# dropbox/lepton

Measured on AMD Instinct MI355X. Metric: encode+decode MB/s (JPEG bytes/sec), bit-exact round trip, higher is better.
Workload: dtype int16/u8 (integer coder, no floating point)

## Files before the change

lepton_amd/csrc/lep_dec4.h:

```cpp
#pragma once
#include "lep_v3.h"
#include "lep_enc3.h"

namespace lep4 {
using namespace lep3;

#if LEP_ON_GPU && defined(LEP_MARKS)
#define LEP_MARK(name) __asm__ volatile("; MARK " name)
#elif LEP_ON_GPU && defined(LEP_PROF)
#define LEP_MARK(name) prof_stamp(lep4::prof_slot(name))
#else
#define LEP_MARK(name) ((void)0)
#endif
#if LEP_ON_GPU && (defined(LEP_DEC4_PAD_VALU) || defined(LEP_DEC4_PAD_SALU) || defined(LEP_DEC4_PAD_LDS))
#define LEP_PAD8(x) x x x x x x x x
WDEV void pad_block(uint32_t seed, const void* lds) {
    (void)seed; (void)lds;
#ifdef LEP_DEC4_PAD_VALU
    { uint32_t o; for (int i = 0; i < LEP_DEC4_PAD_VALU / 8; ++i) __asm__ volatile(LEP_PAD8("v_add_u32 %0, %1, %1\n") : "=v"(o) : "v"(seed)); }
#endif
#ifdef LEP_DEC4_PAD_SALU
    { uint32_t o; const uint32_t u = uni(seed); for (int i = 0; i < LEP_DEC4_PAD_SALU / 8; ++i) __asm__ volatile(LEP_PAD8("s_add_u32 %0, %1, %1\n") : "=s"(o) : "s"(u) : "scc"); }
#endif
#ifdef LEP_DEC4_PAD_LDS
// ... 86 lines not shown
        }
        r.mul = q + (rem ? 1u : 0u);
        r.shift = s - 1;
        return r;
    }
};
WDEV uint32_t mulhi_u32(uint32_t a, uint32_t b) {
#if LEP_ON_GPU
    return __umulhi(a, b);
#else
    return (uint32_t)(((uint64_t)a * b) >> 32);
#endif
}
WDEV int32_t div_by(int32_t n, uint32_t mul, uint32_t shift) {
    const int32_t sign = n >> 31;
    const uint32_t u = ((uint32_t)n ^ (uint32_t)sign) - (uint32_t)sign;
    const uint32_t q = mulhi_u32(u, mul) >> shift;
    return (int32_t)((q ^ (uint32_t)sign) - (uint32_t)sign);
}
WDEV uint32_t bupd_t(uint32_t w, uint32_t obs, const uint32_t* inv24) {
    const uint32_t f = (w & 255) + (obs ^ 1), t = ((w >> 8) & 255) + obs;
    uint32_t nw = f | (t << 8) | ((mul24(f << 8, inv24[f + t]) >> 24) << 16);
    if ((f | t) > 255) {
        const uint32_t f0 = w & 255, t0 = (w >> 8) & 255;
        if ((obs ? f0 : t0) == 1) nw = (w & 0xffff) | ((obs ? 0u : 255u) << 16);
        else {
            const uint32_t f2 = obs ? (1 + f0) >> 1 : 129u, t2 = obs ? 129u : (1 + t0) >> 1;
            nw = f2 | (t2 << 8) | ((mul24(f2 << 8, inv24[f2 + t2]) >> 24) << 16);
        }
    }
    return nw;
}
WDEV uint32_t bupd_u(uint32_t w, uint32_t obs, const uint32_t* inv24) {
    const uint32_t w2 = w + 1u + obs * 255u;
    const uint32_t f = w2 & 255u, t = (w2 >> 8) & 255u;
    if (ucond((f < t ? f : t) == 0)) {
        const uint32_t f0 = w & 255, t0 = (w >> 8) & 255;
        if (ucond((obs ? f0 : t0) == 1)) return (w & 0xffff) | ((obs ? 0u : 255u) << 16);
        const uint32_t f2 = obs ? (1 + f0) >> 1 : 129u, t2 = obs ? 129u : (1 + t0) >> 1;
        return f2 | (t2 << 8) | ((mul24(f2 << 8, inv24[f2 + t2]) >> 24) << 16);
    }
    return (w2 & 0xffffu) | (mul24_low(f, inv24[f + t]) & 0xff0000u);
}

WDEV uint64_t pair64(uint32_t hi, uint32_t lo) {
#if LEP_ON_GPU && !defined(LEP_DEC4_PAIR_OR)
    typedef uint32_t u32x2 __attribute__((ext_vector_type(2)));
    const u32x2 p = {lo, hi};
    return __builtin_bit_cast(uint64_t, p);
#else
    return ((uint64_t)hi << 32) | lo;
#endif
}
struct BoolDec4 {
    uint32_t vhi, vlo;
    int count;
    uint32_t range;
    const uint32_t* words;
    uint32_t first, end;
    uint32_t wi;
    uint32_t raw;

    WDEV uint32_t fetch(uint32_t k) const { return k * 4 < end ? words[k] : 0u; }
    WDEV void refill() {
        const uint32_t lo = wi * 4;
        uint32_t w = __builtin_bswap32(raw);
        int nbits = 32;
        if (lo + 4 > end) w = lo < end ? (w & ~(0xffffffffu >> ((end - lo) * 8))) : 0u;
        if (lo < first) { w <<= (first - lo) * 8; nbits -= (int)(first - lo) * 8; }
        const uint64_t add = ((uint64_t)w << 32) >> (count + 8);
        vhi |= (uint32_t)(add >> 32); vlo |= (uint32_t)add;
        count += nbits;
        ++wi;
        raw = fetch(wi);
    }
    WDEV void init_stream(const uint8_t* p, uint32_t n) {
        const uint32_t mis = (uint32_t)((uintptr_t)p & 3);
        words = reinterpret_cast<const uint32_t*>(p - mis);
        first = mis; end = mis + n;
        vhi = vec(0); vlo = vec(0); count = (int)vec((uint32_t)-8); range = vec(255); wi = 0;
        raw = fetch(0);
        refill();
        get(128);
    }
    WDEV uint32_t get(uint32_t prob) {
#if LEP_ON_GPU
        const uint32_t split = 1 + (__umul24(range - 1, prob) >> 8);
#else
        const uint32_t split = 1 + (((range - 1) * prob) >> 8);
#endif
        if (ucond(count < 0)) refill();
        const uint32_t big = split << 24;
        const uint32_t bit = vhi >= big ? 1u : 0u;
        const uint32_t d = vhi - big;
        vhi = d < vhi ? d : vhi;
        range = bit ? range - split : split;
#ifdef LEP_TRACE_GET
        LEP_TRACE_GET(prob, (int)bit);
#endif
        const int shift = __builtin_clz(range) - 24;
        range <<= shift;
        const uint64_t v = pair64(vhi, vlo) << shift;
        vhi = (uint32_t)(v >> 32); vlo = (uint32_t)v;
        count -= shift;
        return bit;
    }
};

struct BoolDec4S {
    uint32_t vhi, vlo;
    int count;
    uint32_t range;
#ifdef LEP_DEC4_RANGE_LOW
    WDEV void load(const BoolDec4& b) { vhi = uni(b.vhi); vlo = uni(b.vlo); count = (int)uni((uint32_t)b.count); range = uni(b.range); }
    WDEV void store(BoolDec4& b) const { b.vhi = vec(vhi); b.vlo = vec(vlo); b.count = (int)vec((uint32_t)count); b.range = vec(range); }
#else
    WDEV void load(const BoolDec4& b) { vhi = uni(b.vhi); vlo = uni(b.vlo); count = (int)uni((uint32_t)b.count); range = uni(b.range) << 24; }
    WDEV void store(BoolDec4& b) const { b.vhi = vec(vhi); b.vlo = vec(vlo); b.count = (int)vec((uint32_t)count); b.range = vec(range >> 24); }
#endif
    WDEV void refill(BoolDec4& b) {
        const uint32_t lo = b.wi * 4;
        uint32_t w = __builtin_bswap32(uni(b.raw));
        int nbits = 32;
        if (lo + 4 > b.end) w = lo < b.end ? (w & ~(0xffffffffu >> ((b.end - lo) * 8))) : 0u;
        if (lo < b.first) { w <<= (b.first - lo) * 8; nbits -= (int)(b.first - lo) * 8; }
        const uint64_t add = ((uint64_t)w << 32) >> (count + 8);
        vhi |= (uint32_t)(add >> 32); vlo |= (uint32_t)add;
        count += nbits;
        ++b.wi;
        b.raw = b.fetch(b.wi);
    }
    WDEV uint32_t get(BoolDec4& b, uint32_t pk) {
        if (count < 0) refill(b);
#ifdef LEP_DEC4_RANGE_LOW
        const uint32_t split = 1 + (((range - 1) * (pk & 255u)) >> 8);
        const uint32_t big = split << 24;
        uint32_t was = vhi;
        const uint32_t bit = was >= big ? 1u : 0u;
        vhi = bit ? was - big : was;
        range = bit ? range - split : split;
        const int shift = __builtin_clz(range) - 24;
#else
        const uint32_t big = ((uint32_t)(((uint64_t)(range - 0x01000000u) * (uint64_t)(pk << 24)) >> 32) & 0xff000000u) + 0x01000000u;
        uint32_t was = vhi;
        const uint32_t bit = was >= big ? 1u : 0u;
        vhi = bit ? was - big : was;
        range = bit ? range - big : big;
        const int shift = __builtin_clz(range);
#endif
#ifdef LEP_TRACE_GET
        LEP_TRACE_GET(pk & 255u, (int)bit);
#endif
        range <<= shift;
        const uint64_t v = pair64(vhi, vlo) << shift;
        vhi = (uint32_t)(v >> 32); vlo = (uint32_t)v;
        count -= shift;
#if LEP_ON_GPU && !defined(LEP_DEC4_PAIR_OR)
        __asm__ volatile("" : "+s"(was));
        return was >= big ? 1u : 0u;
#else
        return bit;
#endif
    }
};

#ifndef LEP_DEC4_PRIO
#define LEP_DEC4_PRIO 1
#endif
#if LEP_ON_GPU && LEP_DEC4_PRIO
#define LEP_PRIO_SERIAL(on_scalar_unit) __builtin_amdgcn_s_setprio((on_scalar_unit) ? 0 : 1)
#define LEP_PRIO_PARALLEL() __builtin_amdgcn_s_setprio(2)
#else
#define LEP_PRIO_SERIAL(on_scalar_unit) ((void)0)
#define LEP_PRIO_PARALLEL() ((void)0)
#endif
#ifndef LEP_DEC4_SCALAR
#define LEP_DEC4_SCALAR 2
#endif

enum : int32_t { kRowsFresh = 0, kRowsRunning = 1, kRowsFinished = 2, kRowsFailed = 3 };
struct Dec4Resume {
    int32_t state, code;
    uint32_t idx, top;
    uint32_t vhi, vlo;
    int32_t count;
    uint32_t range, wi;
    uint32_t nbins;
    int32_t rows_done[3];
    int32_t fail_component, fail_y, fail_x;
};

struct RowsWalk {
    const Dec4Resume* rec; const uint32_t* lds_save;
    bool fresh;
    uint32_t idx, stop, total;
    int band;
    bool top[3];
    int rows_done[3];
    int state, fail_component, fail_y, fail_x;
};

template <int SCMASK>
struct Dec4WaveT {
    const ImageDev* img;
    uint32_t* model;
    Dec4Shared* sh;
    int comp, ci;
    BoolDec4 bc;
    uint32_t nbins;
#if LEP_ON_GPU && !defined(LEP_COUNT_BINS)
#define LEP_BINS(expr) ((void)0)
#else
#define LEP_BINS(expr) (expr)
#endif
#if LEP_ON_GPU && defined(LEP_PROF)
    uint64_t prof_last;
    unsigned long long* prof_out;
    int prof_cur;
    uint32_t prof_acc[20];
    template <int I> __device__ __forceinline__ void prof_add(uint32_t dt) { if (prof_cur == I) prof_acc[I] += dt; }
    __device__ __forceinline__ void prof_stamp(int slot) {
        const uint64_t t = __builtin_readcyclecounter();
        const uint32_t dt = (uint32_t)(t - prof_last);
        prof_last = t;
        prof_add<0>(dt); prof_add<1>(dt); prof_add<2>(dt); prof_add<3>(dt); prof_add<4>(dt); prof_add<5>(dt); prof_add<6>(dt);
        prof_add<7>(dt); prof_add<8>(dt); prof_add<9>(dt); prof_add<10>(dt); prof_add<11>(dt); prof_add<12>(dt); prof_add<13>(dt);
        prof_add<14>(dt); prof_add<15>(dt); prof_add<16>(dt); prof_add<17>(dt); prof_add<18>(dt);
        prof_cur = slot;
    }
    __device__ __forceinline__ void prof_begin(unsigned long long* out) {
        for (int i = 0; i < 20; ++i) prof_acc[i] = 0;
        prof_out = out; prof_cur = 18; prof_last = __builtin_readcyclecounter();
    }
    __device__ __forceinline__ void prof_end() {
        prof_stamp(18);
        if (threadIdx.x == 0) for (int i = 0; i < 19; ++i) prof_out[i] = prof_acc[i];
    }
#endif

    WDEV void init_tables() {
        LANES(l) {
            sh->r2a[l] = kR2A[l]; sh->a2r[l] = kA2R[l]; sh->nzbin[l] = l < 50 ? kNzBin[l] : 9;
            for (int d = l; d < kSignWords; d += 64) sh->sign[d] = kBranchInit;
            for (int d = l; d < kResDcWords; d += 64) sh->resdc[d] = kBranchInit;
            if (l < (int)(sizeof(NSum) / 4)) { ((uint32_t*)&sh->ns_left)[l] = 0; ((uint32_t*)&sh->ns_above)[l] = 0; }
            for (int d = l; d < 512; d += 64) sh->inv24[d] = inv24_of((uint32_t)d);
            if (l < 32) {
                int j = 0, c = l;
                while (j < 6 && c >= 7 - j) { c -= 7 - j; ++j; }
                sh->cj[l] = (uint8_t)(l < 28 ? j : 7); sh->cn[l] = (uint8_t)(l < 28 ? c + 1 : 0);
            }
        }
        LSYNC();
    }
    WDEV void stage_component(int c) {
        comp = c; ci = c ? 1 : 0;
        LANES(l) {
            sh->q[l] = img->q[c][l];
            sh->thr[l] = img->min_thresh[c][l];
            if (l >= 8) { sh->icos_x[l] = img->icos_x[c][l]; sh->icos_y[l] = img->icos_y[c][l]; }
            if (l < 15) {
                const uint32_t d = l < 7 ? (uint32_t)img->icos_x[c][(l + 1) * 8] : (l < 14 ? (uint32_t)img->icos_y[c][(l - 6) * 8] : (uint32_t)img->q[c][0]);
                const DivBy m = DivBy::of(d < 2 || d > 0x7fffffffu ? 2u : d);
                if (l < 7) sh->icos_x[l] = (int32_t)m.mul;
                else if (l < 14) sh->icos_y[l - 7] = (int32_t)m.mul;
                else { sh->icos_x[7] = (int32_t)m.mul; sh->icos_y[7] = d == 1 ? 32 : (int32_t)m.shift; }
            }
        }
        LSYNC();
    }

    template <bool SC>
    struct Serial {
        Dec4WaveT& w;
        BoolDec4S s;
        WDEV explicit Serial(Dec4WaveT& w_) : w(w_) { if (SC) s.load(w.bc); }
        WDEV void done() { if (SC) s.store(w.bc); }
        static WDEV uint32_t U(uint32_t x) { return SC ? uni(x) : vec(x); }
        static WDEV bool is(bool c) { return SC ? c : ucond(c); }
        WDEV uint32_t get(uint32_t prob) { return SC ? s.get(w.bc, prob) : w.bc.get(prob); }
        WDEV uint32_t bupd(uint32_t word, uint32_t obs) {
            if (!SC) return bupd_u(word, obs, w.sh->inv24);
            const uint32_t w2 = word + 1u + obs * 255u;
            const uint32_t f = w2 & 255u, t = (w2 >> 8) & 255u;
            if ((f < t ? f : t) == 0) {
                const uint32_t f0 = word & 255, t0 = (word >> 8) & 255;
                if ((obs ? f0 : t0) == 1) return (word & 0xffff) | ((obs ? 0u : 255u) << 16);
                const uint32_t f2 = obs ? (1 + f0) >> 1 : 129u, t2 = obs ? 129u : (1 + t0) >> 1;
                return f2 | (t2 << 8) | ((((f2 << 8) * uni(w.sh->inv24[f2 + t2])) >> 24) << 16);
            }
            return (w2 & 0xffffu) | ((f * uni(w.sh->inv24[f + t])) & 0xff0000u);
        }
        WDEV uint32_t global_bin(uint32_t idx) {
            const uint32_t word = U(vload(w.model + idx));
            const uint32_t bit = get(word >> 16);
            const uint32_t nw = bupd(word, bit);
#if LEP_ON_GPU
            if (threadIdx.x == 0) w.model[idx] = nw;
#else
            w.model[idx] = nw;
#endif
            return bit;
        }
        template <int K>
        WDEV int unary_from(uint32_t pk) {
            if (K <= 0) { if (!is(get(pk & 255) != 0)) return 0; }
            if (K <= 1) { if (!is(get((pk >> 8) & 255) != 0)) return 1; }
            if (K <= 2) { if (!is(get((pk >> 16) & 255) != 0)) return 2; }
            if (!is(get(pk >> 24) != 0)) return 3;
            return 4;
        }
        WDEV int unary_tail(uint32_t gbase) {
            int i = 8;
#pragma nounroll
            for (; i < 11; ++i) if (!is(global_bin(row_word(gbase, i)) != 0)) break;
            return i;
        }
        WDEV uint32_t residual(uint32_t pk, int b, uint32_t v) {
            if (b >= 3) v |= get(pk >> 24) << 3;
            if (b >= 2) v |= get((pk >> 16) & 255) << 2;
            if (b >= 1) v |= get((pk >> 8) & 255) << 1;
            if (b >= 0) v |= get(pk & 255);
            return v;
        }
        template <int LEVELS>
        WDEV int tree(const uint32_t* PK, int base) {
            uint32_t pk = U(lepwave::wave_read(PK, base));
            uint32_t n = get(pk & 255);
            pk = U(lepwave::wave_read(PK, base + 1));
            n = (n << 1) | get((pk >> (n * 8)) & 255);
            pk = U(lepwave::wave_read(PK, base + 2));
            n = (n << 1) | get((pk >> (n * 8)) & 255);
#pragma unroll
            for (int d = 3; d < LEVELS; ++d) {
                pk = U(lepwave::wave_read(PK, base + (1 << (d - 2)) + 1 + (int)uni(n >> 2)));
                n = (n << 1) | get((pk >> ((n & 3) * 8)) & 255);
            }
            return (int)uni(n);
        }
    };

    static WDEV U4 vload4(const uint32_t* p) {
#if LEP_ON_GPU
        uintptr_t a = (uintptr_t)p;
        __asm__ volatile("" : "+v"(a));
        return ld4(reinterpret_cast<const uint32_t*>(a));
#else
        return ld4(p);
#endif
    }
    static WDEV uint32_t vload(const uint32_t* p) {
#if LEP_ON_GPU
        uintptr_t a = (uintptr_t)p;
        __asm__ volatile("" : "+v"(a));
        return *reinterpret_cast<const uint32_t*>(a);
#else
        return *p;
#endif
    }
    WDEV void idct_rows() { idct_no_dc(sh); }
    static WDEV int half16(int d) { return (int16_t)d / 2; }

    static WDEV void mask_exp(int i0, int len, int& used, int& bits) {
        int n = imin(len, 10) - i0 + 1;
        n = n < 0 ? 0 : (n > 4 ? 4 : n);
        used = (1 << n) - 1;
        const int z = len - i0;
        bits = (z >= 0 && z < 4) ? (used & ~(1 << z)) : used;
    }
    static WDEV void mask_res(int top, int v, int& used, int& bits) {
        top = top > 3 ? 3 : top;
        used = top < 0 ? 0 : (1 << (top + 1)) - 1;
        bits = v & used;
    }
    static WDEV void mask_tree(int i, int k, int value, int& used, int& bits) {
        const int prefix = value >> (i + 1);
        used = (prefix >> 2) == k ? 1 << (prefix & 3) : 0;
        bits = ((value >> i) & 1) ? used : 0;
    }
    template <int ALWAYS>
    WDEV void adapt_group(U4* W, const int* used, const int* bits) {
        const uint32_t* inv = sh->inv24;
#ifdef LEP_DEC4_ADAPT_BRANCHY
        {
            LV(int, any0);
#define LEP_SLOT0(k, fld)                                                                                             \
            LANES(l) L(any0) = (L(used) >> k) & 1;                                                                    \
            if (lepwave::wave_ballot(any0)) {                                                                         \
                LANES(l) if ((L(used) >> k) & 1) L(W).fld = bupd_t(L(W).fld, (uint32_t)(L(bits) >> k) & 1u, inv);    \
            }
            LEP_SLOT0(0, x) LEP_SLOT0(1, y) LEP_SLOT0(2, z) LEP_SLOT0(3, w)
#undef LEP_SLOT0
            return;
        }
#endif
        LV(int, any); LV(uint32_t, oldw); LV(uint32_t, low);
#ifdef LEP_DEC4_ALWAYS_OVERRIDE
        constexpr int kAlways = LEP_DEC4_ALWAYS_OVERRIDE;
#else
        constexpr int kAlways = ALWAYS;
#endif
#define LEP_SLOT(k, fld)                                                                                              \
        if (!((kAlways >> k) & 1)) { LANES(l) L(any) = (L(used) >> k) & 1; }                                           \
        if (((kAlways >> k) & 1) || lepwave::wave_ballot(any)) {                                                       \
            LANES(l) {                                                                                                \
                const uint32_t w = L(W).fld;                                                                          \
                const uint32_t u1 = ((uint32_t)(L(used) & L(bits)) >> k) & 1u, u0 = ((uint32_t)(L(used) & ~L(bits)) >> k) & 1u;   \
                const uint32_t w2 = w + (u0 | (u1 << 8));                                                             \
                const uint32_t f = w2 & 255u, t = (w2 >> 8) & 255u;                                                   \
                const uint32_t p = mul24_low(f, inv[f + t]);    \
                const uint32_t m = mul24(u0 | u1, 0xff0000u);                                                         \
                L(oldw) = w; L(low) = (f < t ? f : t) + ((u0 | u1) ^ 1u);    \
                L(W).fld = (p & m) | (w2 & ~m);                                                                       \
            }                                                                                                         \
            LANES(l) L(any) = L(low) == 0;                                                                            \
            if (lepwave::wave_ballot(any)) {                                                                          \
                LANES(l) if (L(low) == 0) L(W).fld = bupd_t(L(oldw), (uint32_t)(L(bits) >> k) & 1u, inv);             \
            }                                                                                                         \
        }
        LEP_SLOT(0, x) LEP_SLOT(1, y) LEP_SLOT(2, z) LEP_SLOT(3, w)
#undef LEP_SLOT
    }

    WDEV int round_nz(int nzbin_ctx) {
        LEP_MARK("nz_prefetch");
        LV(U4, W0); LV(uint32_t, a0); LV(uint32_t, PK0);
        LANES(l) {
            uint32_t adr = 0, pk = 0;
            if (l < 17) {
                int i, k;
                if (l < 3) { i = 5 - l; k = 0; } else if (l < 5) { i = 2; k = l - 3; } else if (l < 9) { i = 1; k = l - 5; } else { i = 0; k = l - 9; }
                adr = ctx_nz7(ci, nzbin_ctx) + (uint32_t)i * 32 + (uint32_t)k * 4;
                L(W0) = ld4(model + adr); pk = pack_probs(L(W0));
            }
            L(a0) = adr; L(PK0) = pk;
        }
        LEP_MARK("nz_serial"); LEP_PRIO_SERIAL((SCMASK & 1) != 0);
        int nz;
        {
            Serial<(SCMASK & 1) != 0> sr(*this);
            nz = sr.template tree<6>(PK0, 0);
            sr.done();
            LEP_BINS(nbins += 6);
        }
        LEP_MARK("nz_update"); LEP_PRIO_PARALLEL();
        LV(int, u0); LV(int, b0);
        LANES(l) {
            int u = 0, b = 0;
            if (l < 17) {
                int i, k;
                if (l < 3) { i = 5 - l; k = 0; } else if (l < 5) { i = 2; k = l - 3; } else if (l < 9) { i = 1; k = l - 5; } else { i = 0; k = l - 9; }
                mask_tree(i, k, nz, u, b);
            }
            L(u0) = u; L(b0) = b;
        }
        adapt_group<3>(W0, u0, b0);
        LANES(l) if (L(u0)) st4(model + L(a0), L(W0));
        return nz;
    }

    WDEV void round_77(int& zz_io, int& left_io) {
        Dec4Shared& S = *sh;
        LEP_MARK("77_prefetch");
        const int zz0 = zz_io, left0 = left_io, nb0 = nzbin_of(left0);
        LV(U4, W0); LV(U4, W1); LV(uint32_t, a0); LV(uint32_t, a1); LV(uint32_t, PK0); LV(uint32_t, PK1); LV(int, ok);
        LANES(l) {
            const int pi = l & 15, cand = l >> 4, p = zz0 + pi, nb = nb0 - cand;
            uint32_t adr0 = 0, adr1 = 0, pk0 = 0, pk1 = 0;
            const int valid = p < 49 && nb >= 1 && cand < LEP_DEC4_CANDS && pi >= left0 - nzhi_of(nb < 0 ? 0 : nb);
            if (valid) {
                adr0 = ctx4_exp7(ci, nb, p, S.bsr[p]);
                adr1 = ctx4_res(ci, S.a2r[p], nb);
                L(W0) = ld4(model + adr0);
                pk0 = pack_probs(L(W0));
                L(W1) = ld4(model + adr1); pk1 = pack_probs(L(W1));

            }
            L(a0) = adr0; L(a1) = adr1; L(PK0) = pk0; L(PK1) = pk1; L(ok) = valid;
        }
        LSYNC();
        LEP_MARK("77_serial"); LEP_PRIO_SERIAL((SCMASK & 2) != 0);
        int zz, left = left0, cand = 0;
        const int pi_end = zz0 + 16 < 49 ? 16 : 49 - zz0;
        {
            typedef Serial<(SCMASK & 2) != 0> SR;
            SR sr(*this);
            uint32_t sgw = SR::U(S.sign[ci * 48]);
            int pi = 0;
#pragma nounroll
            for (;;) {
                int lane = pi + 16 * cand;
                const int lane_end = pi_end + 16 * cand;
                uint32_t pkv;
                bool found = false;
#pragma nounroll
                for (;;) {
                    pkv = SR::U(lepwave::wave_read(PK0, lane));
                    LEP_BINS(++nbins);
                    if (SR::is(sr.get(pkv & 255) != 0)) { found = true; break; }
                    if (++lane >= lane_end) break;
                }
                pi = lane - 16 * cand;
                if (!found) break;
                zz = zz0 + pi;
                int len = sr.template unary_from<1>(pkv);
                if (len == 4) {
                    len = 4 + sr.template unary_from<0>(SR::U(pack_probs(vload4(model + ctx4_exp7(ci, nb0 - cand, zz, (int)uni(S.bsr[zz])) + kGS))));
                    if (len == 8) len = sr.unary_tail(ctx4_exp7(ci, nb0 - cand, zz, (int)uni(S.bsr[zz])));
                }
                LEP_BINS(nbins += (uint32_t)(2 * len - (len == 11)));
                const uint32_t pos = sr.get(sgw >> 16);
                sgw = sr.bupd(sgw, pos);
                --left;
                uint32_t v = 1u << (len - 1);
                if (len > 1) {
                    int b = len - 2;
                    if (b >= 4) {
                        const uint32_t rbase = ctx4_res(ci, (int)uni(S.a2r[zz]), nb0 - cand);
#pragma nounroll
                        for (; b >= 4; --b) v |= sr.global_bin(row_word(rbase, b)) << b;
                    }
                    v = sr.residual(SR::U(lepwave::wave_read(PK1, lane)), b, v);
                }
                S.here[zz] = (int16_t)(pos ? (int)v : -(int)v);
                ++pi;
                if (left == 0) break;
                cand = nb0 - nzbin_of(left);
                if (cand >= LEP_DEC4_CANDS || pi >= pi_end) break;
            }
            zz = zz0 + pi;
            sr.done();
            S.sign[ci * 48] = sgw;
        }
        LSYNC();
        LEP_MARK("77_update"); LEP_PRIO_PARALLEL();
        LV(int, nzw);
        LANES(l) L(nzw) = l < 16 && zz0 + l < zz && S.here[zz0 + l] != 0;
        const uint32_t nzmask = (uint32_t)lepwave::wave_ballot(nzw);
        LV(int, u0); LV(int, b0); LV(int, u1); LV(int, b1); LV(int, u2); LV(int, b2);
        LANES(l) {
            int ua = 0, ba = 0, ub = 0, bb = 0, uc = 0, bcc = 0;
            const int pi = l & 15, cand_l = l >> 4, p = zz0 + pi;
            if (L(ok) && p < zz) {
                const int left_at = left0 - __builtin_popcount(nzmask & ((1u << pi) - 1));
                if (left_at > 0 && nb0 - (int)S.nzbin[left_at] == cand_l) {
                    const int cf = S.here[p];
                    const int v = cf < 0 ? -cf : cf, len = bitlen((uint32_t)v);
                    mask_exp(0, len, ua, ba);
                    mask_res(len - 2, v, ub, bb);
                    mask_exp(4, len, uc, bcc);
                }
            }
            L(u0) = ua; L(b0) = ba; L(u1) = ub; L(b1) = bb; L(u2) = uc; L(b2) = bcc;
        }
        adapt_group<3>(W0, u0, b0);
        adapt_group<0>(W1, u1, b1);
        LANES(l) {
            if (L(u0)) st4(model + L(a0), L(W0));
            if (L(u1)) st4(model + L(a1), L(W1));
        }
        if (lepwave::wave_ballot(u2)) {
            LV(U4, W2);
            LANES(l) if (L(u2)) L(W2) = ld4(model + L(a0) + kGS);
            adapt_group<0>(W2, u2, b2);
            LANES(l) if (L(u2)) st4(model + L(a0) + kGS, L(W2));
        }
        LSYNC();
        zz_io = zz; left_io = left;
    }

    WDEV int round_edges(int nz, int eob_x, int eob_y, bool has_left, bool has_above) {
        Dec4Shared& S = *sh;
        LEP_MARK("edge_prefetch");
        LV(U4, W0); LV(U4, W1); LV(U4, W2); LV(uint32_t, a0); LV(uint32_t, a2); LV(uint32_t, PK0); LV(uint32_t, PK1); LV(uint32_t, PK2);
        LV(uint32_t, INFO);
        LANES(l) {
            uint32_t adr0 = 0, adr2 = 0, pk0 = 0, pk1 = 0, pk2 = 0, info = 0;
            if (l < 56) {
                const int e = l >= 28 ? 1 : 0, c = l - e * 28, j = S.cj[c], n = S.cn[c];
                const bool horizontal = e == 0;
                const int coord = horizontal ? j + 1 : (j + 1) * 8;
                const int32_t prior = S.eprior[e * 7 + j];
                const uint32_t ap = prior < 0 ? 0u - (uint32_t)prior : (uint32_t)prior;
                const int bsr = bitlen(ap > 1023 ? 1023 : ap);
                adr0 = ctx4_expx(ci, n, horizontal ? j : j + 7, bsr);
                adr2 = ctx4_res(ci, coord, n);
                L(W0) = ld4(model + adr0); L(W2) = ld4(model + adr2);
                pk0 = pack_probs(L(W0)); pk2 = pack_probs(L(W2));
                L(W1) = U4{0, 0, 0, 0};
                const int16_t p16 = (int16_t)prior;
                const int thr = S.thr[coord];
                const uint32_t tctx = (uint32_t)imin((int)((ap & 0xffff) >> thr), 255);
                info = (uint32_t)((ci * 4 + (p16 == 0 ? 0 : (p16 > 0 ? 1 : 2))) * 12 + bsr) | ((uint32_t)thr << 8) | (tctx << 16) |
                       ((uint32_t)bsr << 24) | ((S.eprior[14] >> (e * 7 + j)) & 1 ? 0x80000000u : 0u);
            } else if (l < 62) {
                const int e = l >= 59 ? 1 : 0, lv = l - 56 - 3 * e;
                adr0 = ctx_nzedge(e == 0, ci, e == 0 ? eob_x : eob_y, (nz + 3) / 7) + (uint32_t)(2 - lv) * 4;
                L(W0) = ld4(model + adr0); pk0 = pack_probs(L(W0));
            }
            L(a0) = adr0; L(a2) = adr2; L(PK0) = pk0; L(PK1) = pk1; L(PK2) = pk2; L(INFO) = info;
        }
        LSYNC();
        LEP_MARK("edge_serial"); LEP_PRIO_SERIAL((SCMASK & 4) != 0);
        int ne[2] = {0, 0}, rc = 0;
        typedef Serial<(SCMASK & 4) != 0> SR;
        SR sr(*this);
#pragma nounroll
        for (int e = 0; e < 2 && !rc; ++e) {
            const bool horizontal = e == 0;
            ne[e] = sr.template tree<3>(PK0, 56 + 3 * e);
            LEP_BINS(nbins += 3);
            int left = ne[e];
            if (!left) continue;
            const int a_off = horizontal ? 50 : 57;
            int lane = e * 28 + left - 1, step = 7;
#pragma nounroll
            for (;;) {
                if (SR::is(left > step)) {
#pragma nounroll
                    for (int j = 7 - step; j < 7 && left; ++j) {
                        const uint32_t info = lepwave::wave_read(INFO, e * 28 + combo_base(j));
                        if (info >> 31) { rc = 43; break; }
                        const int coord = horizontal ? j + 1 : (j + 1) * 8;
                        const uint32_t gb = ctx4_expx(ci, left, horizontal ? j : j + 7, (int)((info >> 24) & 15));
                        int len = 0;
#pragma nounroll
                        for (; len < 11; ++len) if (!SR::is(sr.global_bin(row_word(gb, len)) != 0)) break;
                        LEP_BINS(nbins += (uint32_t)(len ? 2 * len + 1 - (len == 11) : 1));
                        if (!len) continue;
                        const int sslot = (int)(info & 255);
                        const uint32_t sgw = SR::U(S.sign[sslot]);
                        const uint32_t pos = sr.get(sgw >> 16);
                        S.sign[sslot] = sr.bupd(sgw, pos);
                        uint32_t v = 1u << (len - 1);
                        int b = len - 2;
                        const int thr = (int)((info >> 8) & 15);
                        if (b >= thr) {
                            const uint32_t Tt = ctx_thresh(ci, (int)((info >> 16) & 255), imin(len - thr, 7));
                            int sx = 1;
#pragma nounroll
                            for (; b >= thr; --b) {
                                const uint32_t bit = sr.global_bin(Tt + (uint32_t)sx);
                                v |= bit << b;
                                sx = imin((sx << 1) | (int)uni(bit), 127);
                            }
                        }
                        const uint32_t rbase = ctx4_res(ci, coord, left);
#pragma nounroll
                        for (; b >= 0; --b) v |= sr.global_bin(row_word(rbase, b)) << b;
                        S.here[a_off + j] = (int16_t)(pos ? (int)v : -(int)v);
                        --left;
                    }
                    break;
                }
                const uint32_t info = lepwave::wave_read(INFO, lane);
                if (info >> 31) { rc = 43; break; }
                const uint32_t pkv = SR::U(lepwave::wave_read(PK0, lane));
                LEP_BINS(++nbins);
                if (SR::is(sr.get(pkv & 255) != 0)) {
                    const int j = 7 - step;
                    const int coord = horizontal ? j + 1 : (j + 1) * 8;
                    int len = sr.template unary_from<1>(pkv);
                    if (len == 4) {
                        len = 4 + sr.template unary_from<0>(SR::U(pack_probs(vload4(model + ctx4_expx(ci, left, horizontal ? j : j + 7, (int)((info >> 24) & 15)) + kGS))));
                        if (len == 8) len = sr.unary_tail(ctx4_expx(ci, left, horizontal ? j : j + 7, (int)((info >> 24) & 15)));
                    }
                    LEP_BINS(nbins += (uint32_t)(2 * len - (len == 11)));
                    const int sslot = (int)(info & 255);
                    const uint32_t sgw = SR::U(S.sign[sslot]);
                    const uint32_t pos = sr.get(sgw >> 16);
                    S.sign[sslot] = sr.bupd(sgw, pos);
                    uint32_t v = 1u << (len - 1);
                    if (len > 1) {
                        int b = len - 2;
                        const int thr = (int)((info >> 8) & 15);
                        if (b >= thr) {
                            const uint32_t Tt = ctx_thresh(ci, (int)((info >> 16) & 255), imin(len - thr, 7));
                            int sx = 1;
#pragma nounroll
                            for (; b >= thr; --b) {
                                const uint32_t bit = sr.global_bin(Tt + (uint32_t)sx);
                                v |= bit << b;
                                sx = imin((sx << 1) | (int)uni(bit), 127);
                            }
                        }
                        if (b >= 4) {
                            const uint32_t rbase = ctx4_res(ci, coord, left);
#pragma nounroll
                            for (; b >= 4; --b) v |= sr.global_bin(row_word(rbase, b)) << b;
                        }
                        v = sr.residual(SR::U(lepwave::wave_read(PK2, lane)), b, v);
                    }
                    S.here[a_off + j] = (int16_t)(pos ? (int)v : -(int)v);
                    --lane;
                    if (--left == 0) break;
                }
                lane += step;
                if (--step == 0) break;
            }
        }
        sr.done();
        LSYNC();
        if (rc) return rc;
        LEP_MARK("edge_update"); LEP_PRIO_PARALLEL();
        LV(int, enz);
        LANES(l) L(enz) = l >= 50 && S.here[l] != 0;
        const uint64_t em = lepwave::wave_ballot(enz);
        const uint32_t mh = (uint32_t)(em >> 50) & 0x7f, mv = (uint32_t)(em >> 57) & 0x7f;
        const int neh = ne[0], nev = ne[1];
        LV(int, u0); LV(int, b0); LV(int, u1); LV(int, b1); LV(int, u2); LV(int, b2);
        LANES(l) {
            int ua = 0, ba = 0, ub = 0, bb = 0, uc = 0, bcc = 0;
            if (l < 56) {
                const int e = l >= 28 ? 1 : 0, c = l - e * 28, j = S.cj[c], n = S.cn[c];
                const uint32_t mk = e ? mv : mh;
                const int left_at = (e ? nev : neh) - __builtin_popcount(mk & ((1u << j) - 1));
                if (left_at == n) {
                    const int cf = S.here[(e ? 57 : 50) + j];
                    const int v = cf < 0 ? -cf : cf, len = bitlen((uint32_t)v);
                    mask_exp(0, len, ua, ba);
                    mask_exp(4, len, ub, bb);
                    mask_res(imin(len - 2, (int)S.thr[e ? (j + 1) * 8 : j + 1] - 1), v, uc, bcc);
                }
            } else if (l < 62) {
                const int e = l >= 59 ? 1 : 0, lv = l - 56 - 3 * e;
                mask_tree(2 - lv, 0, e ? nev : neh, ua, ba);
            }
            L(u0) = ua; L(b0) = ba; L(u1) = ub; L(b1) = bb; L(u2) = uc; L(b2) = bcc;
        }
        adapt_group<3>(W0, u0, b0);
        LANES(l) if (L(u0)) st4(model + L(a0), L(W0));
        if (lepwave::wave_ballot(u1)) {
            LANES(l) if (L(u1)) L(W1) = ld4(model + L(a0) + kGS);
            adapt_group<0>(W1, u1, b1);
            LANES(l) if (L(u1)) st4(model + L(a0) + kGS, L(W1));
        }
        if (lepwave::wave_ballot(u2)) {
            adapt_group<0>(W2, u2, b2);
            LANES(l) if (L(u2)) st4(model + L(a2), L(W2));
        }
        LSYNC();
        return 0;
    }

    WDEV void round_dc(int pred, int a, int b17, int sctx) {
        Dec4Shared& S = *sh;
        LEP_MARK("dc_prefetch");
        LV(U4, W0); LV(uint32_t, a0); LV(uint32_t, PK0); LV(uint32_t, RW);
        LANES(l) {
            uint32_t adr = 0, pk = 0, rw = 0;
            if (l < 3) { adr = ctx_expdc(a, b17) + (uint32_t)l * 4; L(W0) = ld4(model + adr); pk = pack_probs(L(W0)); }
            else if (l < 13) rw = S.resdc[a * 12 + (l - 3)];
            L(a0) = adr; L(PK0) = pk; L(RW) = rw;
        }
        LEP_MARK("dc_serial"); LEP_PRIO_SERIAL((SCMASK & 8) != 0);
        const int sslot = ci * 48 + sctx;
        typedef Serial<(SCMASK & 8) != 0> SR;
        SR sr(*this);
        int len = sr.template unary_from<0>(SR::U(lepwave::wave_read(PK0, 0)));
        if (len == 4) {
            len += sr.template unary_from<0>(SR::U(lepwave::wave_read(PK0, 1)));
            if (len == 8) {
                uint32_t pk = SR::U(lepwave::wave_read(PK0, 2));
#pragma nounroll
                for (; len < 11; ++len) { if (!SR::is(sr.get(pk & 255) != 0)) break; pk >>= 8; }
            }
        }
        LEP_BINS(nbins += (uint32_t)(len ? 2 * len + 1 - (len == 11) : 1));
        uint32_t v = 0, pos = 1;
        if (len) {
            const uint32_t sgw = SR::U(S.sign[sslot]);
            pos = sr.get(sgw >> 16);
            S.sign[sslot] = sr.bupd(sgw, pos);
            v = 1u << (len - 1);
#pragma nounroll
            for (int i = len - 2; i >= 0; --i) v |= sr.get(SR::U(lepwave::wave_read(RW, 3 + i)) >> 16) << i;
        }
        sr.done();
        v = vec(v);
        int d = (int16_t)(pos ? (int)v : -(int)v);
        int dc = d + pred;
        dc = dc < -1024 ? dc + 2049 : dc;
        dc = dc > 1024 ? dc - 2049 : dc;
        S.here[49] = (int16_t)dc;
        LSYNC();
        LEP_MARK("dc_update"); LEP_PRIO_PARALLEL();
        LV(uint32_t, VV); LV(int, u0); LV(int, b0);
        LANES(l) L(VV) = v;
        LANES(l) {
            int u = 0, b = 0;
            if (l < 3) mask_exp(l * 4, len, u, b);
            L(u0) = u; L(b0) = b;
        }
        adapt_group<7>(W0, u0, b0);
        LANES(l) {
            if (L(u0)) st4(model + L(a0), L(W0));
            if (l >= 3 && l < 13 && l - 3 <= len - 2) S.resdc[a * 12 + (l - 3)] = bupd_t(L(RW), (L(VV) >> (l - 3)) & 1u, S.inv24);
        }
        LSYNC();
    }

    WDEV int decode_block(bool has_left, bool has_above) {
        Dec4Shared& S = *sh;
        LEP_MARK("prologue");
        LANES(l) {
            S.here[l] = 0;
            if (l < 49) {
                int prior;
                if (has_left && has_above) prior = (uint16_t)((iabs(S.left[l]) + iabs(S.above[l])) * 13 + 6 * iabs(S.aleft[l])) >> 5;
                else if (has_left) prior = (int16_t)iabs(S.left[l]);
                else if (has_above) prior = (int16_t)iabs(S.above[l]);
                else prior = 0;
                S.bsr[l] = (uint8_t)bitlen((uint32_t)imin(iabs(prior), 1023));
            }
        }
        int nzctx = 0;
        if (has_left && has_above) nzctx = (S.ns_above.nz + S.ns_left.nz + 2) / 4;
        else if (has_above) nzctx = (S.ns_above.nz + 1) / 2;
        else if (has_left) nzctx = (S.ns_left.nz + 1) / 2;
        const int nzbin_ctx = (int)uni((uint32_t)nzbin_of(nzctx));
        LSYNC();

        const int nz = round_nz(nzbin_ctx);
        if (nz > 49) return 7;
        {
            int zz = 0, left = nz;
#pragma nounroll
            while (zz < 49 && left > 0) round_77(zz, left);
        }
        LEP_MARK("lakhani");
        int eob_x, eob_y;
        {
            LV(int, tx); LV(int, ty); LV(int, badf);
            LANES(l) {
                int ex = 0, ey = 0, bad = 0;
                if (l < 49 && S.here[l] != 0) { const int coord = S.a2r[l]; ex = coord & 7; ey = coord >> 3; }
                if (l < 14) {
                    const bool hz = l < 7;
                    const int j = hz ? l : l - 7;
                    const int coord = hz ? j + 1 : (j + 1) * 8;
                    int32_t prior = 0;
                    if (hz ? has_above : has_left) {
                        const int16_t* nbr = hz ? S.above : S.left;
                        const int32_t* icos = hz ? S.icos_x + coord * 8 : S.icos_y + coord;
                        const int step = hz ? 8 : 1;
                        if (icos[0] != 0) {
                            uint32_t acc = (uint32_t)(int32_t)nbr[S.r2a[coord]] * (uint32_t)icos[0];
                            for (int i = 1; i < 8; ++i) {
                                int32_t xi = S.here[S.r2a[coord + i * step]], ai = nbr[S.r2a[coord + i * step]];
                                int32_t term = (i & 1) ? xi + ai : xi - ai;
                                acc -= (uint32_t)icos[i] * (uint32_t)term;
// ... 180 lines not shown
```

lepton_amd/csrc/lep_wave.h:

```cpp
#pragma once
#include <stdint.h>

#if defined(__HIPCC__)
#define LEP_ON_GPU 1
#define LEP_NL 1
#define LEP_LI(l) 0
static __device__ __forceinline__ int lep_lane_now() { int v = (int)(threadIdx.x & 63); __asm__ volatile("" : "+v"(v)); return v; }
#define LANES(l) for (int l = lep_lane_now(), lep_once_ = 1; lep_once_; lep_once_ = 0)
#define WSYNC() __syncthreads()
#define LSYNC() do { __builtin_amdgcn_fence(__ATOMIC_SEQ_CST, "wavefront"); __builtin_amdgcn_wave_barrier(); } while (0)
#define WDEV __device__ __forceinline__
#else
#define LEP_ON_GPU 0
#define LEP_NL 64
#define LEP_LI(l) (l)
static inline int lep_lane_id(int i) { __asm__ volatile("" : "+r"(i)); return i; }
#define LANES(l) for (int lep_i_ = 0; lep_i_ < 64; ++lep_i_) for (int l = lep_lane_id(lep_i_), lep_once_ = 1; lep_once_; lep_once_ = 0)
#define WSYNC() ((void)0)
#define LSYNC() ((void)0)
#define WDEV inline
#endif

#define LV(T, name) T name[LEP_NL]
#define L(name) name[LEP_LI(l)]
// ... 43 lines not shown
#else
    int s = 0;
    for (int i = 0; i < 64; ++i) { int v = in[i]; out[i] = s; s += v; }
    return s;
#endif
}
WDEV int wave_sum(const int* in) {
#if LEP_ON_GPU
    return __builtin_amdgcn_readlane(wave_incl_sum(in[0]), 63);
#else
    int s = 0;
    for (int i = 0; i < 64; ++i) s += in[i];
    return s;
#endif
}

WDEV int wave_max(const int* in) {
#if LEP_ON_GPU
    return __builtin_amdgcn_readlane(wave_incl_max(in[0]), 63);
#else
    int m = in[0];
    for (int i = 1; i < 64; ++i) m = in[i] > m ? in[i] : m;
    return m;
#endif
}

WDEV void wave_prefix_max(const int* in, int* out) {
#if LEP_ON_GPU
    out[0] = wave_incl_max(in[0]);
#else
    int m = in[0];
    for (int i = 0; i < 64; ++i) { m = in[i] > m ? in[i] : m; out[i] = m; }
#endif
}
WDEV void wave_suffix_min(const int* in, int* out) {
#if LEP_ON_GPU
    const int rev = (63 - (int)(threadIdx.x & 63)) * 4;
    const int r = __builtin_amdgcn_ds_bpermute(rev, -in[0]);
    out[0] = -__builtin_amdgcn_ds_bpermute(rev, wave_incl_max(r));
#else
    int m = in[63];
    for (int i = 63; i >= 0; --i) { m = in[i] < m ? in[i] : m; out[i] = m; }
#endif
}

WDEV uint32_t wave_read(const uint32_t* v, int src) {
#if LEP_ON_GPU
    return (uint32_t)__builtin_amdgcn_readlane((int)v[0], src);
#else
    return v[src];
#endif
}

WDEV void wave_write(uint32_t* v, int dst, uint32_t value) {
#if LEP_ON_GPU
    v[0] = (int)(threadIdx.x & 63) == dst ? value : v[0];
#else
    v[dst] = value;
#endif
}

WDEV void wave_select(uint32_t* v, uint64_t m, uint32_t value) {
#if LEP_ON_GPU
    __asm__("v_cndmask_b32_e64 %0, %0, %1, %2" : "+v"(v[0]) : "v"(value), "s"(m));
#else
    for (int i = 0; i < 64; ++i) if ((m >> i) & 1ull) v[i] = value;
#endif
}
WDEV int popc64(uint64_t m) { return __builtin_popcountll(m); }

#if LEP_ON_GPU
template <class T> WDEV T gld(const T* p) { return *(const __attribute__((address_space(1))) T*)(uintptr_t)p; }
template <class T> WDEV void gst(T* p, const T& v) { *(__attribute__((address_space(1))) T*)(uintptr_t)p = v; }
#else
template <class T> WDEV T gld(const T* p) { return *p; }
template <class T> WDEV void gst(T* p, const T& v) { *p = v; }
#endif

WDEV int mbcnt(uint64_t m, int l) {
#if LEP_ON_GPU
    (void)l;
    return (int)__builtin_amdgcn_mbcnt_hi((uint32_t)(m >> 32), __builtin_amdgcn_mbcnt_lo((uint32_t)m, 0u));
#else
    return __builtin_popcountll(m & ((1ull << l) - 1));
#endif
}

}
```

Before: 1578.

## Batch bool-decoder refills per bin group and adapt model words one per lane

The arithmetic decoder now refills whenever fewer than 24 bits remain, with one check before each group of up to three or four bins (unary runs, residuals, tree levels), instead of testing for refill before every bin. Separately, model adaptation after the nz, 7x7, edge and DC rounds no longer updates whole 4-word groups per lane. Each lane instead gathers its single word via ds_bpermute, adapts it, and stores it with a scalar store. Both aim to shorten the serial decode critical path and the vector update work. The cost is extra cross-lane permutes and more complex lane-mapping logic, which must remain bit-exact.

```diff
diff --git a/lepton_amd/csrc/lep_dec4.h b/lepton_amd/csrc/lep_dec4.h
--- a/lepton_amd/csrc/lep_dec4.h
+++ b/lepton_amd/csrc/lep_dec4.h
@@ -162,6 +162,9 @@
     return ((uint64_t)hi << 32) | lo;
 #endif
 }
+#ifndef LEP_DEC4_REFILL_GROUPS
+#define LEP_DEC4_REFILL_GROUPS 1
+#endif
 struct BoolDec4 {
     uint32_t vhi, vlo;
     int count;
@@ -191,15 +194,24 @@
         vhi = vec(0); vlo = vec(0); count = (int)vec((uint32_t)-8); range = vec(255); wi = 0;
         raw = fetch(0);
         refill();
-        get(128);
-    }
-    WDEV uint32_t get(uint32_t prob) {
+        ensure();
+        get_raw(128);
+    }
+    WDEV void ensure() {
+#if LEP_DEC4_REFILL_GROUPS
+        if (ucond(count < 24)) refill();
+#endif
+    }
+    WDEV uint32_t get(uint32_t prob) { ensure(); return get_raw(prob); }
+    WDEV uint32_t get_raw(uint32_t prob) {
 #if LEP_ON_GPU
         const uint32_t split = 1 + (__umul24(range - 1, prob) >> 8);
 #else
         const uint32_t split = 1 + (((range - 1) * prob) >> 8);
 #endif
+#if !LEP_DEC4_REFILL_GROUPS
         if (ucond(count < 0)) refill();
+#endif
         const uint32_t big = split << 24;
         const uint32_t bit = vhi >= big ? 1u : 0u;
         const uint32_t d = vhi - big;
@@ -240,8 +252,20 @@
         ++b.wi;
         b.raw = b.fetch(b.wi);
     }
-    WDEV uint32_t get(BoolDec4& b, uint32_t pk) {
+    WDEV void ensure(BoolDec4& b) {
+#if LEP_DEC4_REFILL_GROUPS
+        if (count < 24) refill(b);
+#else
+        (void)b;
+#endif
+    }
+    WDEV uint32_t get(BoolDec4& b, uint32_t pk) { ensure(b); return get_raw(b, pk); }
+    WDEV uint32_t get_raw(BoolDec4& b, uint32_t pk) {
+#if !LEP_DEC4_REFILL_GROUPS
         if (count < 0) refill(b);
+#else
+        (void)b;
+#endif
 #ifdef LEP_DEC4_RANGE_LOW
         const uint32_t split = 1 + (((range - 1) * (pk & 255u)) >> 8);
         const uint32_t big = split << 24;
@@ -286,6 +310,10 @@
 #endif
 #ifndef LEP_DEC4_SCALAR
 #define LEP_DEC4_SCALAR 2
+#endif
+
+#ifndef LEP_DEC4_WORD_PER_LANE
+#define LEP_DEC4_WORD_PER_LANE 1
 #endif
 
 enum : int32_t { kRowsFresh = 0, kRowsRunning = 1, kRowsFinished = 2, kRowsFailed = 3 };
@@ -389,6 +417,8 @@
         static WDEV uint32_t U(uint32_t x) { return SC ? uni(x) : vec(x); }
         static WDEV bool is(bool c) { return SC ? c : ucond(c); }
         WDEV uint32_t get(uint32_t prob) { return SC ? s.get(w.bc, prob) : w.bc.get(prob); }
+        WDEV void ensure() { if (SC) s.ensure(w.bc); else w.bc.ensure(); }
+        WDEV uint32_t get_raw(uint32_t prob) { return SC ? s.get_raw(w.bc, prob) : w.bc.get_raw(prob); }
         WDEV uint32_t bupd(uint32_t word, uint32_t obs) {
             if (!SC) return bupd_u(word, obs, w.sh->inv24);
             const uint32_t w2 = word + 1u + obs * 255u;
@@ -412,12 +442,14 @@
 #endif
             return bit;
         }
-        template <int K>
+        template <int K, bool ENSURE = true>
         WDEV int unary_from(uint32_t pk) {
-            if (K <= 0) { if (!is(get(pk & 255) != 0)) return 0; }
-            if (K <= 1) { if (!is(get((pk >> 8) & 255) != 0)) return 1; }
-            if (K <= 2) { if (!is(get((pk >> 16) & 255) != 0)) return 2; }
-            if (!is(get(pk >> 24) != 0)) return 3;
+            static_assert(ENSURE || K >= 1, "four bins need a refill test of their own");
+            if (ENSURE) ensure();
+            if (K <= 0) { if (!is(get_raw(pk & 255) != 0)) return 0; }
+            if (K <= 1) { if (!is(get_raw((pk >> 8) & 255) != 0)) return 1; }
+            if (K <= 2) { if (!is(get_raw((pk >> 16) & 255) != 0)) return 2; }
+            if (!is(get_raw(pk >> 24) != 0)) return 3;
             return 4;
         }
         WDEV int unary_tail(uint32_t gbase) {
@@ -427,24 +459,27 @@
             return i;
         }
         WDEV uint32_t residual(uint32_t pk, int b, uint32_t v) {
-            if (b >= 3) v |= get(pk >> 24) << 3;
-            if (b >= 2) v |= get((pk >> 16) & 255) << 2;
-            if (b >= 1) v |= get((pk >> 8) & 255) << 1;
-            if (b >= 0) v |= get(pk & 255);
+            if (b >= 3) { ensure(); v |= get_raw(pk >> 24) << 3; }
+            if (b >= 2) v |= get_raw((pk >> 16) & 255) << 2;
+            if (b >= 1) v |= get_raw((pk >> 8) & 255) << 1;
+            if (b >= 0) v |= get_raw(pk & 255);
             return v;
         }
         template <int LEVELS>
         WDEV int tree(const uint32_t* PK, int base) {
+            static_assert(LEVELS <= 6, "one refill test per three levels");
             uint32_t pk = U(lepwave::wave_read(PK, base));
-            uint32_t n = get(pk & 255);
+            ensure();
+            uint32_t n = get_raw(pk & 255);
             pk = U(lepwave::wave_read(PK, base + 1));
-            n = (n << 1) | get((pk >> (n * 8)) & 255);
+            n = (n << 1) | get_raw((pk >> (n * 8)) & 255);
             pk = U(lepwave::wave_read(PK, base + 2));
-            n = (n << 1) | get((pk >> (n * 8)) & 255);
+            n = (n << 1) | get_raw((pk >> (n * 8)) & 255);
+            if (LEVELS > 3) ensure();
 #pragma unroll
             for (int d = 3; d < LEVELS; ++d) {
                 pk = U(lepwave::wave_read(PK, base + (1 << (d - 2)) + 1 + (int)uni(n >> 2)));
-                n = (n << 1) | get((pk >> ((n & 3) * 8)) & 255);
+                n = (n << 1) | get_raw((pk >> ((n & 3) * 8)) & 255);
             }
             return (int)uni(n);
         }
@@ -532,6 +567,39 @@
 #undef LEP_SLOT
     }
 
+    WDEV void adapt_words(uint32_t* W, const int* use, const int* obs) {
+        const uint32_t* inv = sh->inv24;
+        LV(int, wrapped); LV(uint32_t, oldw);
+        LANES(l) {
+            const uint32_t w = L(W);
+            const uint32_t u = (uint32_t)L(use), u1 = u & (uint32_t)L(obs), u0 = u & ~(uint32_t)L(obs);
+            const uint32_t w2 = w + (u0 | (u1 << 8));
+            const uint32_t f = w2 & 255u, t = (w2 >> 8) & 255u;
+            const uint32_t p = mul24_low(f, inv[f + t]);
+            const uint32_t m = mul24(u, 0xff0000u);
+            L(oldw) = w; L(wrapped) = (f < t ? f : t) + (u ^ 1u) == 0;
+            L(W) = (p & m) | (w2 & ~m);
+        }
+        if (lepwave::wave_ballot(wrapped)) {
+            LANES(l) if (L(wrapped)) L(W) = bupd_t(L(oldw), (uint32_t)L(obs), inv);
+        }
+    }
+    static WDEV void regroup(const U4* G, const int* src, const int* slot, uint32_t* out) {
+        LV(uint32_t, c0); LV(uint32_t, c1); LV(uint32_t, c2); LV(uint32_t, c3);
+        LV(uint32_t, g0); LV(uint32_t, g1); LV(uint32_t, g2); LV(uint32_t, g3);
+        LANES(l) { L(c0) = L(G).x; L(c1) = L(G).y; L(c2) = L(G).z; L(c3) = L(G).w; }
+        lepwave::wave_gather(c0, src, g0); lepwave::wave_gather(c1, src, g1);
+        lepwave::wave_gather(c2, src, g2); lepwave::wave_gather(c3, src, g3);
+        LANES(l) { const int k = L(slot); L(out) = k == 0 ? L(g0) : (k == 1 ? L(g1) : (k == 2 ? L(g2) : L(g3))); }
+    }
+    WDEV void adapt_regrouped(const U4* G, const uint32_t* adr, const int* src, const int* slot, const int* use, const int* obs) {
+        LV(uint32_t, Wd); LV(uint32_t, ad);
+        regroup(G, src, slot, Wd);
+        lepwave::wave_gather(adr, src, ad);
+        adapt_words(Wd, use, obs);
+        LANES(l) if (L(use)) model[L(ad) + (uint32_t)L(slot)] = L(Wd);
+    }
+
     WDEV int round_nz(int nzbin_ctx) {
         LEP_MARK("nz_prefetch");
         LV(U4, W0); LV(uint32_t, a0); LV(uint32_t, PK0);
@@ -554,6 +622,16 @@
             LEP_BINS(nbins += 6);
         }
         LEP_MARK("nz_update"); LEP_PRIO_PARALLEL();
+#if LEP_DEC4_WORD_PER_LANE
+        {
+            LV(int, src); LV(int, slot); LV(int, use); LV(int, ob);
+            LANES(l) {
+                const int t = l < 6 ? l : 0, i = 5 - t, prefix = nz >> (i + 1);
+                L(src) = ((0x953210 >> (4 * t)) & 15) + (prefix >> 2); L(slot) = prefix & 3; L(use) = l < 6; L(ob) = (nz >> i) & 1;
+            }
+            adapt_regrouped(W0, a0, src, slot, use, ob);
+        }
+#else
         LV(int, u0); LV(int, b0);
         LANES(l) {
             int u = 0, b = 0;
@@ -566,6 +644,7 @@
         }
         adapt_group<3>(W0, u0, b0);
         LANES(l) if (L(u0)) st4(model + L(a0), L(W0));
+#endif
         return nz;
     }
 
@@ -573,7 +652,10 @@
         Dec4Shared& S = *sh;
         LEP_MARK("77_prefetch");
         const int zz0 = zz_io, left0 = left_io, nb0 = nzbin_of(left0);
-        LV(U4, W0); LV(U4, W1); LV(uint32_t, a0); LV(uint32_t, a1); LV(uint32_t, PK0); LV(uint32_t, PK1); LV(int, ok);
+        LV(U4, W0); LV(U4, W1); LV(uint32_t, a0); LV(uint32_t, a1); LV(uint32_t, PK0); LV(uint32_t, PK1);
+#if !LEP_DEC4_WORD_PER_LANE
+        LV(int, ok);
+#endif
         LANES(l) {
             const int pi = l & 15, cand = l >> 4, p = zz0 + pi, nb = nb0 - cand;
             uint32_t adr0 = 0, adr1 = 0, pk0 = 0, pk1 = 0;
@@ -586,7 +668,10 @@
                 L(W1) = ld4(model + adr1); pk1 = pack_probs(L(W1));
 
             }
-            L(a0) = adr0; L(a1) = adr1; L(PK0) = pk0; L(PK1) = pk1; L(ok) = valid;
+            L(a0) = adr0; L(a1) = adr1; L(PK0) = pk0; L(PK1) = pk1;
+#if !LEP_DEC4_WORD_PER_LANE
+            L(ok) = valid;
+#endif
         }
         LSYNC();
         LEP_MARK("77_serial"); LEP_PRIO_SERIAL((SCMASK & 2) != 0);
@@ -613,7 +698,7 @@
                 pi = lane - 16 * cand;
                 if (!found) break;
                 zz = zz0 + pi;
-                int len = sr.template unary_from<1>(pkv);
+                int len = sr.template unary_from<1, false>(pkv);
                 if (len == 4) {
                     len = 4 + sr.template unary_from<0>(SR::U(pack_probs(vload4(model + ctx4_exp7(ci, nb0 - cand, zz, (int)uni(S.bsr[zz])) + kGS))));
                     if (len == 8) len = sr.unary_tail(ctx4_exp7(ci, nb0 - cand, zz, (int)uni(S.bsr[zz])));
@@ -648,6 +733,28 @@
         LANES(l) L(nzw) = l < 16 && zz0 + l < zz && S.here[zz0 + l] != 0;
         const uint32_t nzmask = (uint32_t)lepwave::wave_ballot(nzw);
         LV(int, u0); LV(int, b0); LV(int, u1); LV(int, b1); LV(int, u2); LV(int, b2);
+#if LEP_DEC4_WORD_PER_LANE
+        LV(int, src); LV(int, slot);
+        LANES(l) {
+            int s = l, ua = 0, oa = 0, ub = 0, ob = 0, uc = 0, bcc = 0;
+            const int pi = l & 15, k = l >> 4, p = zz0 + pi;
+            if (p < zz) {
+                const int left_at = left0 - __builtin_popcount(nzmask & ((1u << pi) - 1));
+                const int c = left_at > 0 ? nb0 - (int)S.nzbin[left_at] : LEP_DEC4_CANDS;
+                if (c < LEP_DEC4_CANDS) {
+                    const int cf = S.here[p];
+                    const int v = cf < 0 ? -cf : cf, len = bitlen((uint32_t)v);
+                    s = pi + 16 * c;
+                    ua = k <= len; oa = len != k;
+                    ub = k <= len - 2; ob = (v >> k) & 1;
+                    if (c == k) mask_exp(4, len, uc, bcc);
+                }
+            }
+            L(src) = s; L(slot) = k; L(u0) = ua; L(b0) = oa; L(u1) = ub; L(b1) = ob; L(u2) = uc; L(b2) = bcc;
+        }
+        adapt_regrouped(W0, a0, src, slot, u0, b0);
+        if (lepwave::wave_ballot(u1)) adapt_regrouped(W1, a1, src, slot, u1, b1);
+#else
         LANES(l) {
             int ua = 0, ba = 0, ub = 0, bb = 0, uc = 0, bcc = 0;
             const int pi = l & 15, cand_l = l >> 4, p = zz0 + pi;
@@ -669,6 +776,7 @@
             if (L(u0)) st4(model + L(a0), L(W0));
             if (L(u1)) st4(model + L(a1), L(W1));
         }
+#endif
         if (lepwave::wave_ballot(u2)) {
             LV(U4, W2);
             LANES(l) if (L(u2)) L(W2) = ld4(model + L(a0) + kGS);
@@ -770,7 +878,7 @@
                 if (SR::is(sr.get(pkv & 255) != 0)) {
                     const int j = 7 - step;
                     const int coord = horizontal ? j + 1 : (j + 1) * 8;
-                    int len = sr.template unary_from<1>(pkv);
+                    int len = sr.template unary_from<1, false>(pkv);
                     if (len == 4) {
                         len = 4 + sr.template unary_from<0>(SR::U(pack_probs(vload4(model + ctx4_expx(ci, left, horizontal ? j : j + 7, (int)((info >> 24) & 15)) + kGS))));
                         if (len == 8) len = sr.unary_tail(ctx4_expx(ci, left, horizontal ? j : j + 7, (int)((info >> 24) & 15)));
@@ -818,7 +926,10 @@
         const uint64_t em = lepwave::wave_ballot(enz);
         const uint32_t mh = (uint32_t)(em >> 50) & 0x7f, mv = (uint32_t)(em >> 57) & 0x7f;
         const int neh = ne[0], nev = ne[1];
-        LV(int, u0); LV(int, b0); LV(int, u1); LV(int, b1); LV(int, u2); LV(int, b2);
+        LV(int, u1); LV(int, b1); LV(int, u2); LV(int, b2);
+#if !LEP_DEC4_WORD_PER_LANE
+        LV(int, u0); LV(int, b0);
+#endif
         LANES(l) {
             int ua = 0, ba = 0, ub = 0, bb = 0, uc = 0, bcc = 0;
             if (l < 56) {
@@ -828,18 +939,50 @@
                 if (left_at == n) {
                     const int cf = S.here[(e ? 57 : 50) + j];
                     const int v = cf < 0 ? -cf : cf, len = bitlen((uint32_t)v);
+#if !LEP_DEC4_WORD_PER_LANE
                     mask_exp(0, len, ua, ba);
+#endif
                     mask_exp(4, len, ub, bb);
                     mask_res(imin(len - 2, (int)S.thr[e ? (j + 1) * 8 : j + 1] - 1), v, uc, bcc);
                 }
-            } else if (l < 62) {
+            }
+#if !LEP_DEC4_WORD_PER_LANE
+            else if (l < 62) {
                 const int e = l >= 59 ? 1 : 0, lv = l - 56 - 3 * e;
                 mask_tree(2 - lv, 0, e ? nev : neh, ua, ba);
             }
-            L(u0) = ua; L(b0) = ba; L(u1) = ub; L(b1) = bb; L(u2) = uc; L(b2) = bcc;
-        }
+            L(u0) = ua; L(b0) = ba;
+#else
+            (void)ua; (void)ba;
+#endif
+            L(u1) = ub; L(b1) = bb; L(u2) = uc; L(b2) = bcc;
+        }
+#if LEP_DEC4_WORD_PER_LANE
+        {
+            LV(int, src); LV(int, slot); LV(int, use); LV(int, ob);
+            LANES(l) {
+                int s = l, k = l & 3, u = 0, o = 0;
+                if (l < 56) {
+                    const int q = l >> 2, e = q >= 7 ? 1 : 0, j = q - 7 * e;
+                    const int left_at = (e ? nev : neh) - __builtin_popcount((e ? mv : mh) & ((1u << j) - 1));
+                    if (left_at >= 1 && left_at <= 7 - j) {
+                        const int cf = S.here[(e ? 57 : 50) + j];
+                        const int v = cf < 0 ? -cf : cf, len = bitlen((uint32_t)v);
+                        s = e * 28 + ((j * (15 - j)) >> 1) + left_at - 1;
+                        u = k <= len; o = len != k;
+                    }
+                } else if (l < 62) {
+                    const int e = l >= 59 ? 1 : 0, i = 2 - (l - 56 - 3 * e), value = e ? nev : neh;
+                    k = (value >> (i + 1)) & 3; u = 1; o = (value >> i) & 1;
+                }
+                L(src) = s; L(slot) = k; L(use) = u; L(ob) = o;
+            }
+            adapt_regrouped(W0, a0, src, slot, use, ob);
+        }
+#else
         adapt_group<3>(W0, u0, b0);
         LANES(l) if (L(u0)) st4(model + L(a0), L(W0));
+#endif
         if (lepwave::wave_ballot(u1)) {
             LANES(l) if (L(u1)) L(W1) = ld4(model + L(a0) + kGS);
             adapt_group<0>(W1, u1, b1);
@@ -872,8 +1015,9 @@
             len += sr.template unary_from<0>(SR::U(lepwave::wave_read(PK0, 1)));
             if (len == 8) {
                 uint32_t pk = SR::U(lepwave::wave_read(PK0, 2));
-#pragma nounroll
-                for (; len < 11; ++len) { if (!SR::is(sr.get(pk & 255) != 0)) break; pk >>= 8; }
+                sr.ensure();
+#pragma nounroll
+                for (; len < 11; ++len) { if (!SR::is(sr.get_raw(pk & 255) != 0)) break; pk >>= 8; }
             }
         }
         LEP_BINS(nbins += (uint32_t)(len ? 2 * len + 1 - (len == 11) : 1));
@@ -895,8 +1039,29 @@
         S.here[49] = (int16_t)dc;
         LSYNC();
         LEP_MARK("dc_update"); LEP_PRIO_PARALLEL();
-        LV(uint32_t, VV); LV(int, u0); LV(int, b0);
+        LV(uint32_t, VV);
         LANES(l) L(VV) = v;
+#if LEP_DEC4_WORD_PER_LANE
+        {
+            LV(int, src); LV(int, slot); LV(int, use); LV(int, ob); LV(uint32_t, Wd); LV(uint32_t, ad); LV(uint32_t, rg);
+            LANES(l) {
+                int s = l, k = 0, u = 0, o = 0;
+                if (l < 11) { s = l >> 2; k = l & 3; u = l <= len; o = len != l; }
+                else if (l < 21) { s = l - 8; u = l - 11 <= len - 2; o = (int)((L(VV) >> (l - 11)) & 1u); }
+                L(src) = s; L(slot) = k; L(use) = u; L(ob) = o;
+            }
+            regroup(W0, src, slot, Wd);
+            lepwave::wave_gather(RW, src, rg);
+            lepwave::wave_gather(a0, src, ad);
+            LANES(l) if (l >= 11) L(Wd) = L(rg);
+            adapt_words(Wd, use, ob);
+            LANES(l) if (L(use)) {
+                if (l < 11) model[L(ad) + (uint32_t)L(slot)] = L(Wd);
+                else S.resdc[a * 12 + (l - 11)] = L(Wd);
+            }
+        }
+#else
+        LV(int, u0); LV(int, b0);
         LANES(l) {
             int u = 0, b = 0;
             if (l < 3) mask_exp(l * 4, len, u, b);
@@ -907,6 +1072,7 @@
             if (L(u0)) st4(model + L(a0), L(W0));
             if (l >= 3 && l < 13 && l - 3 <= len - 2) S.resdc[a * 12 + (l - 3)] = bupd_t(L(RW), (L(VV) >> (l - 3)) & 1u, S.inv24);
         }
+#endif
         LSYNC();
     }
 
diff --git a/lepton_amd/csrc/lep_wave.h b/lepton_amd/csrc/lep_wave.h
--- a/lepton_amd/csrc/lep_wave.h
+++ b/lepton_amd/csrc/lep_wave.h
@@ -119,6 +119,14 @@
 #endif
 }
 
+WDEV void wave_gather(const uint32_t* v, const int* src, uint32_t* out) {
+#if LEP_ON_GPU
+    out[0] = (uint32_t)__builtin_amdgcn_ds_bpermute(src[0] << 2, (int)v[0]);
+#else
+    for (int i = 0; i < 64; ++i) out[i] = v[src[i] & 63];
+#endif
+}
+
 WDEV void wave_write(uint32_t* v, int dst, uint32_t value) {
 #if LEP_ON_GPU
     v[0] = (int)(threadIdx.x & 63) == dst ? value : v[0];
```

New measurement: 1635, median of 6. +3.6%, better.
